# ChuWeiEr/GravInv3DHMC

Measured on AMD Instinct MI355X. Metric: HMC leapfrog steps/sec + G·ρ achieved HBM GB/s at 1/2/4/8 GPUs, higher is better.
Workload: dtype f64

## Files before the change

gravinv3dhmc_amd/_lib.py:

```python
import ctypes as C
import os

import numpy as np

_HERE = os.path.dirname(os.path.abspath(__file__))
LIB_PATH = os.environ.get("GRAVHMC_LIB") or os.path.join(_HERE, "libgravhmc.so")

GH_OK, GH_ERR_ARG, GH_ERR_HIP, GH_ERR_NOMEM, GH_ERR_OVERFLOW, GH_ERR_UNSUPPORTED, GH_ERR_COMM = \
    0, -1, -2, -3, -4, -5, -6
CELL_PRISM, CELL_TESSEROID, CELL_PRISM_TF, CELL_PRISM_COMP, CELL_TESSEROID_COMP, CELL_PRISM_JOINT = 0, 1, 2, 3, 4, 5
CELL_PRISM_MULTI = 6
CELL_PRISM_MVI = 7
CELL_PRISM_MVI_DATA = 8
CELL_TESS_MVI_DATA = 9
CELL_TESSEROID_MULTI = 10
BCOMP_TF, BCOMP_BX, BCOMP_BY, BCOMP_BZ = range(4)
BCOMPONENTS = {"tf": BCOMP_TF, "bx": BCOMP_BX, "by": BCOMP_BY, "bz": BCOMP_BZ}
BCOMP_MAX = 4
MULTI_MAX = 11
COMP_POTENTIAL, COMP_GEOID, COMP_GX, COMP_GY, COMP_GZ, COMP_GXX, COMP_GXY, COMP_GXZ, COMP_GYY, COMP_GYZ, COMP_GZZ = \
    range(11)
COMPONENTS = {"potential": COMP_POTENTIAL, "geoid": COMP_GEOID, "gx": COMP_GX, "gy": COMP_GY, "gz": COMP_GZ,
              "gxx": COMP_GXX, "gxy": COMP_GXY, "gxz": COMP_GXZ, "gyy": COMP_GYY, "gyz": COMP_GYZ, "gzz": COMP_GZZ}
REG_KINDS = {"Damping": 0, "Smoothness": 1, "MS": 2, "TV": 3}
# ... 111 lines not shown
    "gh_shard_init_callback": (C.c_int, [_ctx, C.c_void_p, C.c_void_p, C.c_int, C.c_int, _i64, _i64]),
    "gh_shard_init_rows": (C.c_int, [_ctx, C.c_void_p, C.c_int, C.c_int, _i64, _i64]),
    "gh_shard_init_rows_callback": (C.c_int, [_ctx, C.c_void_p, C.c_void_p, C.c_int, C.c_int, _i64, _i64]),
    "gh_shard_allreduce": (C.c_int, [_ctx, _dp, _i64]),
    "gh_rng_create": (C.c_int, [C.POINTER(C.c_void_p), C.c_uint32]),
    "gh_rng_destroy": (None, [C.c_void_p]),
    "gh_rng_set_threads": (C.c_int, [C.c_void_p, C.c_int]),
    "gh_host_cores": (C.c_int, []),
    "gh_rng_set_state": (C.c_int, [C.c_void_p, C.POINTER(C.c_uint32), C.c_int, C.c_int, C.c_double]),
    "gh_rng_get_state": (C.c_int, [C.c_void_p, C.POINTER(C.c_uint32), C.POINTER(C.c_int), C.POINTER(C.c_int),
                                   C.POINTER(C.c_double)]),
    "gh_rng_draw_trajectories": (C.c_int, [C.c_void_p, C.c_int, C.c_int, C.c_int, _i64, C.c_double,
                                           C.POINTER(C.c_int), _dp, _dp]),
    "gh_format_row_fixed8": (C.c_int64, [_dp, _i64, C.c_char_p, _i64]),
    "gh_measure_stream_read": (C.c_int, [_ctx, C.c_int, C.c_int, C.POINTER(C.c_double)]),
    "gh_profile_enable": (C.c_int, [_ctx, C.c_int]),
    "gh_fold_info": (C.c_int, [_ctx, C.POINTER(C.c_int), C.POINTER(C.c_int), C.POINTER(_i64), C.POINTER(C.c_double),
                               C.POINTER(C.c_double)]),
    "gh_fold_detect": (C.c_int, [_i64, _dp, _dp, _dp, _i64, _dp, C.POINTER(C.c_int), C.POINTER(C.c_int)]),
    "gh_fold_pair_info": (C.c_int, [_ctx, C.POINTER(C.c_int), C.POINTER(C.c_int), C.POINTER(_i64), C.POINTER(_i64),
                                    C.POINTER(_i64)]),
    "gh_fold_detect_pair": (C.c_int, [_i64, _dp, _dp, _dp, _i64, _dp, C.POINTER(C.c_int), C.POINTER(C.c_int),
                                      C.POINTER(C.c_int), C.POINTER(_i64), C.POINTER(C.c_int)]),
    "gh_profile_read": (C.c_int, [_ctx, C.POINTER(C.c_double), C.POINTER(_i64),
                                  C.POINTER(_i64)]),
    "gh_set_translation_invariant": (C.c_int, [_ctx, C.c_int]),
    "gh_translation_invariant_info": (C.c_int, [_ctx] + [C.POINTER(C.c_int)] * 6 + [C.POINTER(_i64), C.POINTER(C.c_double),
                                                                                   C.POINTER(C.c_double)]),
    "gh_translation_invariant_table": (C.c_int, [_ctx, _dp]),
    "gh_lattice_detect": (C.c_int, [_i64, _dp, _dp, _dp, _i64, _dp] + [C.POINTER(C.c_int)] * 5),
}

ALLREDUCE_FN = C.CFUNCTYPE(C.c_int, C.c_void_p, _dp, _i64)

_LIB = None


class GravHmcError(RuntimeError):
    pass


def load():
    global _LIB
    if _LIB is None:
        if not os.path.exists(LIB_PATH):
            raise GravHmcError(
# ... 41 lines not shown
```

gravinv3dhmc_amd/csrc/fold.hip.h:

```cpp
#pragma once

namespace ghk {

struct FoldArgs {
    const double *S;
    const int *obs_img;
    const int *cell_orbit;
    int nF, ldF;
    int64_t n_orb;
    int64_t orb_per_team;
    int n_pp;
    int64_t N;
};

typedef const d2 __attribute__((address_space(1))) *gconst_d2ptr;

__global__ void __launch_bounds__(256) fold_build_kernel(const double *G, int64_t ld, FoldArgs f, double *S,
                                                         unsigned long long *dev_bits)
{
    __shared__ double red[2][4];
    const int64_t o = blockIdx.x;
    const int n = 4 * f.ldF;
    int co[4];
#pragma unroll
// ... 266 lines not shown
            const int e = k * TT + tid;
            const double p2 = __shfl_xor(acc[k][1].x, 1, WAVE), p3 = __shfl_xor(acc[k][1].y, 1, WAVE);
            const double tA = acc[k][0].x + p2, tB = acc[k][0].y + p3;
            const int i = e >> 1;
            if (e < n2 && i < f.nF) {
                const int m2 = 2 * (tid & 1);
                out[f.obs_img[4 * i + m2]] = tA;
                out[f.obs_img[4 * i + m2 + 1]] = tB;
                ds += tA;
                ds += tB;
            }
        }
        for (int64_t e = f.N + tid; e < a.ld; e += TT) out[e] = 0.0;
        if (a.dsum) {
            const double t = block_allreduce_sum(ds, scratch, NW);
            if (tid == 0) a.dsum[blockIdx.x] = t;
        }
    }
}


struct FoldPairArgs {
    const int *wtab;
    const int *obs_img_tau;
    int64_t n_work, work_per_team;
};
constexpr int FOLD_PAIR_W = 16;
constexpr int FOLD_PSLOT = 64;

__global__ void __launch_bounds__(256) fold_pair_mean_kernel(FoldArgs f, const int *row_tau, const int *orb_tau, double *S,
                                                             unsigned long long *dev_bits)
{
    __shared__ double red[2][4];
    const int64_t o = blockIdx.x;
    const int ot = orb_tau[o];
    const int64_t o2 = ot >> 2;
    const int co = ot & 3;
    const int n = 4 * f.nF;
    const int64_t ldb = 4 * (int64_t)f.ldF;
    double dev = 0.0, amax = 0.0;
    if (o <= o2) {
        for (int e = threadIdx.x; e < n; e += blockDim.x) {
            const int k = e & 3, rt = row_tau[e >> 2];
            const int ks = ((k & 1) << 1) | (k >> 1);
            const int e2 = (rt & ~3) | (ks ^ co ^ (rt & 3));
            if (o < o2 || e < e2) {
                const double u = S[o * ldb + e], v = S[o2 * ldb + e2];
                const double m = (u + v) * 0.5;
                S[o * ldb + e] = m;
                S[o2 * ldb + e2] = m;
                dev = fmax(dev, fabs(u - m));
// ... 17 lines not shown
    if (threadIdx.x == 0) {
        for (int w = 1; w < (int)(blockDim.x >> 6); ++w) {
            dev = fmax(dev, red[0][w]);
            amax = fmax(amax, red[1][w]);
        }
        const double rel = amax > 0.0 ? dev / amax : 0.0;
        atomicMax(dev_bits, (unsigned long long)__double_as_longlong(rel));
    }
}

template <int ROWS>
struct FoldPairCol {
    d2 v[ROWS][2];
    int j;
    int jn, on;
    bool live;
    double cv;
};

template <int ROWS>
__global__ void __launch_bounds__(512) fold_pair_sweep_kernel(SweepArgs a, FoldArgs f, FoldPairArgs p)
{
    constexpr int TT = 512, NW = 8;
    extern __shared__ __attribute__((aligned(16))) double smem[];
    double *rF = smem;
    double *rT = smem + 4 * f.nF;
    double *scratch = smem + 8 * f.nF;

    const int tid = threadIdx.x;
    const int lane = tid & 63;
    const int wave = tid >> 6;
    const int mode = a.mode;

    if (mode & SW_ADJ) {
        for (int e = tid; e < 4 * f.nF; e += TT) {
            rF[e] = a.r[f.obs_img[e]];
            rT[e] = a.r[p.obs_img_tau[e]];
        }
    }
    __syncthreads();

    const int64_t wb = (int64_t)blockIdx.x * p.work_per_team;
    int64_t wend = wb + p.work_per_team;
    if (wend > p.n_work) wend = p.n_work;
    const int cnt = wb < wend ? (int)(wend - wb) : 0;

    d2 acc[ROWS][2], accT[ROWS][2];
#pragma unroll
    for (int k = 0; k < ROWS; ++k) acc[k][0] = acc[k][1] = accT[k][0] = accT[k][1] = d2{0.0, 0.0};
    double pp = 0.0;

    const int row_last = (ROWS - 1) * TT + tid;
    const bool last_in = row_last < f.nF;
    unsigned voff = (unsigned)tid * 32u;
    unsigned coff_last = (unsigned)(row_last < f.ldF ? row_last : f.ldF - 1) * 32u;
    const int lrow_last = last_in ? row_last : f.nF - 1;

    const int hl = (lane >> 3) & 3, ql = lane & 7, sl = lane >> 5;
    const double *in_base = ql == FOLD_IN_P      ? a.p_in
                            : ql == FOLD_IN_GREG ? a.greg
                            : ql == FOLD_IN_HI   ? a.high
                            : ql == FOLD_IN_LO   ? a.low
                            : ql == FOLD_IN_PN   ? a.pn_in
                            : (ql == FOLD_IN_GACC && (mode & SW_GACC)) ? a.g_out
                                                                       : a.x_in;
    const int lastc = cnt - 1;
    auto item = [&](int i) -> int64_t { return wb + (i < lastc ? i : lastc); };
    auto load_col = [&](FoldPairCol<ROWS> &c, int64_t w_after) {
        const int jn = p.wtab[FOLD_PAIR_W * w_after + (lane >> 3)];
        const int on = p.wtab[FOLD_PAIR_W * w_after + 8];
        const int64_t o = __builtin_amdgcn_readfirstlane(c.on);
        const unsigned long long col = (unsigned long long)(f.S + o * (int64_t)(4 * f.ldF));
#pragma unroll
        for (int k = 0; k < ROWS - 1; ++k) {
            unsigned long long colk = col + (unsigned long long)k * TT * 32u;
            asm volatile("" : "+s"(colk));
            asm volatile("" : "+v"(voff));
            c.v[k][0] = __builtin_nontemporal_load(reinterpret_cast<gconst_d2ptr>(colk + voff));
            c.v[k][1] = __builtin_nontemporal_load(reinterpret_cast<gconst_d2ptr>(colk + voff) + 1);
        }
        asm volatile("" : "+v"(coff_last));
        c.v[ROWS - 1][0] = __builtin_nontemporal_load(reinterpret_cast<gconst_d2ptr>(col + coff_last));
        c.v[ROWS - 1][1] = __builtin_nontemporal_load(reinterpret_cast<gconst_d2ptr>(col + coff_last) + 1);
        asm volatile("" : "+v"(c.jn)::"memory");
        c.live = c.jn >= 0;
        c.j = c.live ? c.jn : ~c.jn;
        c.cv = in_base[c.j];
        c.jn = jn;
        c.on = on;
    };

    auto row_fma = [](const d2 v0, const d2 v1, const d2 wa, const d2 wb2, d2 &t01, d2 &t23) {
        t01.x += v0.x * wa.x;
        t01.x += v0.y * wa.y;
        t01.x += v1.x * wb2.x;
        t01.x += v1.y * wb2.y;
        t01.y += v0.x * wa.y;
        t01.y += v0.y * wa.x;
        t01.y += v1.x * wb2.y;
        t01.y += v1.y * wb2.x;
        t23.x += v0.x * wb2.x;
        t23.x += v0.y * wb2.y;
        t23.x += v1.x * wa.x;
        t23.x += v1.y * wa.y;
        t23.y += v0.x * wb2.y;
        t23.y += v0.y * wb2.x;
        t23.y += v1.x * wa.y;
        t23.y += v1.y * wa.x;
    };

    auto process = [&](const FoldPairCol<ROWS> &cur, int it) {
        double xl = cur.cv;
        const double pl = dpp_from_up<FOLD_IN_P>(cur.cv);
        if (mode & SW_ADJ) {
            const d2 *r2 = reinterpret_cast<const d2 *>(rF), *t2 = reinterpret_cast<const d2 *>(rT);
            d2 ua = d2{0.0, 0.0}, ub = ua, uta = ua, utb = ua;
#pragma unroll
            for (int k = 0; k < ROWS; ++k) {
                if (k < ROWS - 1 || last_in) {
                    const int row = k < ROWS - 1 ? k * TT + tid : lrow_last;
                    row_fma(cur.v[k][0], cur.v[k][1], r2[2 * row], r2[2 * row + 1], ua, ub);
                    row_fma(cur.v[k][0], cur.v[k][1], t2[2 * row], t2[2 * row + 1], uta, utb);
                }
            }
            const bool odd = (lane & 1) != 0, hi2 = (lane & 2) != 0;
            const double u[4] = {ua.x, ua.y, ub.x, ub.y}, ut[4] = {uta.x, uta.y, utb.x, utb.y};
            double b[4];
#pragma unroll
            for (int q = 0; q < 4; ++q) b[q] = (odd ? ut[q] : u[q]) + dpp_mov<0xb1>(odd ? u[q] : ut[q]);
            double s0 = (hi2 ? b[2] : b[0]) + dpp_mov<0x4e>(hi2 ? b[0] : b[2]);
            double s1 = (hi2 ? b[3] : b[1]) + dpp_mov<0x4e>(hi2 ? b[1] : b[3]);
            s0 = dpp_add<0x114, 0xf>(s0);
            s0 = dpp_add<0x118, 0xf>(s0);
            s1 = dpp_add<0x114, 0xf>(s1);
            s1 = dpp_add<0x118, 0xf>(s1);
            s0 += __shfl_xor(s0, 16, WAVE);
            s1 += __shfl_xor(s1, 16, WAVE);
            s0 += __shfl_xor(s0, 32, WAVE);
            s1 += __shfl_xor(s1, 32, WAVE);
            double *slot = scratch + (it & 1) * FOLD_PSLOT;
            if (lane >= 12 && lane < 16) {
                const int c = lane - 12;
                *reinterpret_cast<d2 *>(slot + wave * 8 + 4 * (c & 1) + 2 * (c >> 1)) = d2{s0, s1};
            }
            __syncthreads();
            double sv = slot[lane];
            sv = dpp_add<0x118, 0xf>(sv);
            sv += __shfl_xor(sv, 16, WAVE);
            sv += __shfl_xor(sv, 32, WAVE);
// ... 22 lines not shown
            if (mode & SW_PFIN) {
                const double pz = cur.live ? pf : 0.0;
#pragma unroll
                for (int h = 0; h < 8; ++h) {
                    const double q = readlane_d(pz, 8 * h);
                    pp += q * q;
                }
            }
            if (tid < 64 && ql == 0 && cur.live) {
                const int j = cur.j;
                if (mode & SW_GOUT) a.g_out[j] = (mode & SW_GACC) ? dpp_from_up<FOLD_IN_GACC>(cur.cv) + g : g;
                if (mode & SW_UPD) {
                    a.p_out[j] = pv;
                    a.x_out[j] = xl;
                } else if ((mode & SW_PFIN) && !(mode & SW_SPEC)) {
                    a.p_out[j] = pv;
                }
            }
        }
        if (mode & SW_FWD) {
            const double xz = cur.live ? xl : 0.0;
            const d2 xa = d2{readlane_d(xz, 0), readlane_d(xz, 8)}, xb = d2{readlane_d(xz, 16), readlane_d(xz, 24)};
            const d2 ya = d2{readlane_d(xz, 32), readlane_d(xz, 40)}, yb = d2{readlane_d(xz, 48), readlane_d(xz, 56)};
#pragma unroll
            for (int k = 0; k < ROWS; ++k) {
                row_fma(cur.v[k][0], cur.v[k][1], xa, xb, acc[k][0], acc[k][1]);
                row_fma(cur.v[k][0], cur.v[k][1], ya, yb, accT[k][0], accT[k][1]);
            }
        }
#pragma unroll
        for (int k = 0; k < ROWS; ++k) {
            asm volatile("" ::"v"(cur.v[k][0]));
            asm volatile("" ::"v"(cur.v[k][1]));
        }
    };

    if (cnt > 0) {
        FoldPairCol<ROWS> b0, b1;
        b0.jn = p.wtab[FOLD_PAIR_W * item(0) + (lane >> 3)];
        b0.on = p.wtab[FOLD_PAIR_W * item(0) + 8];
        b1.jn = p.wtab[FOLD_PAIR_W * item(1) + (lane >> 3)];
        b1.on = p.wtab[FOLD_PAIR_W * item(1) + 8];
        load_col(b0, item(2));
        int i = 0;
        for (;;) {
            load_col(b1, item(i + 3));
            process(b0, i);
            if (++i >= cnt) break;
            load_col(b0, item(i + 3));
            process(b1, i);
            if (++i >= cnt) break;
        }
    }

    if ((mode & SW_PFIN) && tid == 0) {
        a.pp_part[blockIdx.x] = pp;
        for (int t = (int)(blockIdx.x + gridDim.x); t < f.n_pp; t += (int)gridDim.x) a.pp_part[t] = 0.0;
    }

    if (mode & SW_FWD) {
        double *out = a.slab + (int64_t)blockIdx.x * a.ld;
        double ds = 0.0;
#pragma unroll
        for (int k = 0; k < ROWS; ++k) {
            const int i = k * TT + tid;
            if (i < f.nF) {
                const int4 oi = reinterpret_cast<const int4 *>(f.obs_img)[i];
                out[oi.x] = acc[k][0].x;
                out[oi.y] = acc[k][0].y;
                out[oi.z] = acc[k][1].x;
                out[oi.w] = acc[k][1].y;
                ds += acc[k][0].x;
                ds += acc[k][0].y;
                ds += acc[k][1].x;
                ds += acc[k][1].y;
            }
        }
        for (int64_t e = f.N + tid; e < a.ld; e += TT) out[e] = 0.0;
        __syncthreads();
#pragma unroll
        for (int k = 0; k < ROWS; ++k) {
            const int i = k * TT + tid;
            if (i < f.nF) {
                const int4 oi = reinterpret_cast<const int4 *>(p.obs_img_tau)[i];
                out[oi.x] += accT[k][0].x;
                out[oi.y] += accT[k][0].y;
                out[oi.z] += accT[k][1].x;
                out[oi.w] += accT[k][1].y;
                ds += accT[k][0].x;
                ds += accT[k][0].y;
                ds += accT[k][1].x;
                ds += accT[k][1].y;
            }
        }
        if (a.dsum) {
            const double t = block_allreduce_sum(ds, scratch, NW);
            if (tid == 0) a.dsum[blockIdx.x] = t;
        }
    }
}

}
```

gravinv3dhmc_amd/csrc/gravhmc.hip:

```cpp
#include "../../include/gravhmc.h"
#include "kernels.hip.h"
#include "batch.hip.h"
#include "bscg.hip.h"
#include "exchange.hip.h"
#include "resident.hip.h"
#include "resbatch.hip.h"
#include "teamsweep.hip.h"
#include "mfbatch.hip.h"
#include "batchteam.hip.h"
#include "lonsym.hip.h"
#include "lonsymh.hip.h"
#include "lonres.hip.h"
#include "lonsymw.hip.h"
#include "fold.hip.h"
#include "lattice.hip.h"
#include "poststream.hip.h"
#include "tessmag.hip.h"

#include <dlfcn.h>
#include <rccl/rccl.h>

#include <algorithm>
#include <array>
#include <atomic>
// ... 2407 lines not shown
    return GH_OK;
}

int gh_fold_detect_pair(int64_t N, const double *x, const double *y, const double *z, int64_t M, const double *bounds6,
                        int *obs_tau, int *cell_tau, int *work, int64_t *n_work, int *pair_reason)
{
    if (N < 0 || M < 0 || !x || !y || !z || !bounds6 || !obs_tau || !cell_tau || !work || !n_work || !pair_reason)
        return GH_ERR_ARG;
    std::vector<int> oi, co, ot, ct, rt, qt, wk;
    *n_work = 0;
    *pair_reason = GH_FOLD_PAIR_NO_FOLD;
    const int rc = fold_detect_host(N, x, y, z, M, bounds6, oi, co);
    if (rc != GH_FOLD_ON) return rc;
    *pair_reason = fold_pair_detect_host(N, x, y, z, M, bounds6, oi, co, ot, ct, rt, qt, wk);
    if (*pair_reason == GH_FOLD_PAIR_ON) {
        std::copy(ot.begin(), ot.end(), obs_tau);
        std::copy(ct.begin(), ct.end(), cell_tau);
        std::copy(wk.begin(), wk.end(), work);
        *n_work = (int64_t)(wk.size() / 2);
    }
    return rc;
}

int gh_fold_detect(int64_t N, const double *x, const double *y, const double *z, int64_t M, const double *bounds6,
                   int *obs_img, int *cell_orbit)
{
    if (N < 0 || M < 0 || !x || !y || !z || !bounds6 || !obs_img || !cell_orbit) return GH_ERR_ARG;
    std::vector<int> oi, co;
    const int rc = fold_detect_host(N, x, y, z, M, bounds6, oi, co);
    if (rc == GH_FOLD_ON) {
        std::copy(oi.begin(), oi.end(), obs_img);
        std::copy(co.begin(), co.end(), cell_orbit);
    }
    return rc;
}

int gh_profile_read(gh_ctx *c, double *sweep_ms, int64_t *sweep_launches, int64_t *bytes_per_sweep)
{
    if (!c) return GH_ERR_ARG;
    HIPCHK(c, hipSetDevice(c->device));
    HIPCHK(c, hipStreamSynchronize(c->stream));
    const int64_t full = c->N * c->M * (int64_t)sizeof(double);
    int64_t maxb = c->prof_res_evals > 0 ? full : 0;
    for (size_t i = 0; i < c->ev_used / 2; ++i) maxb = std::max(maxb, c->ev_bytes[i]);
    double ms = (c->prof_res_evals > 0 && maxb == full) ? c->prof_ms_acc : 0.0;
    int64_t timed = (c->prof_res_evals > 0 && maxb == full) ? c->prof_res_evals : 0;
// ... 23 lines not shown
```

gravinv3dhmc_amd/csrc/host_ctx.h:

```cpp
#pragma once

static thread_local std::string g_create_error;

struct LonSymHost;
struct LatticeHost;

struct DevBuf {
    void *p = nullptr;
    size_t bytes = 0;
};

struct ExchangeGuard {
    unsigned *abort_w = nullptr;
    unsigned seen[4] = {0, 0, 0, 0};
    unsigned tag = 0, tagE = 0, ltag = 0;
    std::vector<DevBuf> grans;
    bool dirty = false;
    bool inflight = false;
    int aborts = 0;
};

struct BatchSet { double *X, *GREG, *D, *Rt; };

struct gh_ctx {
// ... 291 lines not shown
    uint64_t G_gen = 0;
    struct Fold {
        int detected = 0;
        int reason = GH_FOLD_UNDECIDED;
        uint64_t gen = ~0ull;
        bool valid = false;
        int nF = 0, ldF = 0;
        int64_t n_orb = 0;
        std::vector<int> obs_img, cell_orbit;
        int *obs_img_d = nullptr, *cell_orbit_d = nullptr;
        double *S = nullptr;
        double *zeros = nullptr;
        unsigned long long *dev_bits = nullptr;
        int ept2 = 0, grid = 0;
        int64_t orb_per_team = 0;
        size_t lds = 0;
        double max_dev = 0.0, build_ms = 0.0;
        int64_t launches = 0;
        bool exact = false;
        bool pair_detected = false, pair_on = false;
        int pair_reason = GH_FOLD_PAIR_UNDECIDED;
        int64_t n_work = 0, n_pairs = 0, work_per_team = 0;
        int pair_rows = 0;
        int *wtab_d = nullptr, *obs_img_tau_d = nullptr, *row_tau_d = nullptr, *orb_tau_d = nullptr;
    } fd;

    struct Pinned {
        char *base;
        size_t bytes;
    };
    std::vector<Pinned> pinned;

    double *ring = nullptr, *ring_mean = nullptr, *ring_sd = nullptr;
    int ring_K = 0, ring_next = 0;
    int64_t ring_count = 0;

    struct PostStream {
        bool on = false;
        int slot = 0;
        int64_t from = 0, count = 0;
        ghk::PostState d = {};
        double *lo = nullptr, *hi = nullptr, *iw = nullptr;
        double *row = nullptr;
        double *out = nullptr;
        double *qout = nullptr;
        size_t qout_n = 0;
        int64_t n[16] = {}, K[16] = {};
// ... 114 lines not shown
```

gravinv3dhmc_amd/csrc/host_fold.h:

```cpp
#pragma once


namespace fold_detail {

struct Axis {
    std::vector<double> lo, hi;
    double tol = 0.0;
    void build(std::vector<double> v, double t)
    {
        tol = t;
        std::sort(v.begin(), v.end());
        for (double x : v) {
            if (lo.empty() || x - hi.back() > tol) {
                lo.push_back(x);
                hi.push_back(x);
            } else {
                hi.back() = x;
            }
        }
    }
    int find(double x) const
    {
        const size_t k = (size_t)(std::upper_bound(lo.begin(), lo.end(), x + tol) - lo.begin());
        if (k == 0) return -1;
// ... 230 lines not shown
            if (tau[(size_t)tau[(size_t)i]] != i) return false;
            const int at = pos[(size_t)tau[(size_t)i]] ^ (((g & 1) << 1) | (g >> 1));
            if (g == 0) rt[e >> 2] = at;
            if (rt[e >> 2] != at) return false;
        }
        return true;
    };
    if (!rows(obs_img, obs_tau, row_tau)) return GH_FOLD_PAIR_OBS;
    if (!rows(cell_orbit, cell_tau, orb_tau)) return GH_FOLD_PAIR_CELLS;
    work.clear();
    for (size_t o = 0; o < orb_tau.size(); ++o) {
        const int o2 = orb_tau[o] >> 2;
        if (o2 == (int)o) {
            work.push_back((int)o);
            work.push_back(-1);
        } else if ((int)o < o2) {
            work.push_back((int)o);
            work.push_back(o2);
        }
    }
    return GH_FOLD_PAIR_ON;
}

static int fold_pair_tables(gh_ctx *c, const double *ox, const double *oy, const double *oz, const double *b6)
{
    gh_ctx::Fold &f = c->fd;
    std::vector<int> obs_tau, cell_tau, row_tau, orb_tau, work;
    f.pair_on = false;
    f.n_work = f.n_pairs = 0;
    f.pair_reason = fold_pair_detect_host(c->N, ox, oy, oz, c->M, b6, f.obs_img, f.cell_orbit, obs_tau, cell_tau, row_tau,
                                          orb_tau, work);
    f.pair_detected = f.pair_reason == GH_FOLD_PAIR_ON;
    if (!f.pair_detected) return GH_OK;
    f.pair_reason = GH_FOLD_PAIR_UNDECIDED;
    f.n_work = (int64_t)(work.size() / 2);
    std::vector<int> wtab((size_t)f.n_work * ghk::FOLD_PAIR_W, 0), oit((size_t)c->N);
    for (int64_t w = 0; w < f.n_work; ++w) {
        const int o = work[2 * (size_t)w], o2 = work[2 * (size_t)w + 1];
        int *t = wtab.data() + w * ghk::FOLD_PAIR_W;
        for (int h = 0; h < 4; ++h) {
            t[h] = f.cell_orbit[4 * (size_t)o + h];
            t[4 + h] = o2 >= 0 ? cell_tau[(size_t)t[h]] : ~t[h];
        }
        t[8] = o;
        f.n_pairs += o2 >= 0;
    }
    for (size_t e = 0; e < oit.size(); ++e) oit[e] = obs_tau[(size_t)f.obs_img[e]];
    auto up = [&](int **d, const std::vector<int> &h, size_t cap) -> int {
        TRY(dalloc(c, d, cap, false));
        HIPCHK(c, hipMemcpyAsync(*d, h.data(), sizeof(int) * h.size(), hipMemcpyHostToDevice, c->stream));
        return GH_OK;
    };
    TRY(up(&f.wtab_d, wtab, (size_t)f.n_orb * ghk::FOLD_PAIR_W));
    TRY(up(&f.obs_img_tau_d, oit, (size_t)c->N));
    TRY(up(&f.row_tau_d, row_tau, (size_t)f.nF));
    TRY(up(&f.orb_tau_d, orb_tau, (size_t)f.n_orb));
    HIPCHK(c, hipStreamSynchronize(c->stream));
    return GH_OK;
}

static int fold_detect(gh_ctx *c)
{
    gh_ctx::Fold &f = c->fd;
    f.detected = -1;
    f.valid = false;
    f.gen = ~0ull;
    f.reason = GH_FOLD_NOT_GZ;
    f.pair_detected = f.pair_on = false;
    f.pair_reason = GH_FOLD_PAIR_NO_FOLD;
    if (c->cell_kind != GH_CELL_PRISM || c->joint || c->mf || !c->G) return GH_OK;
    std::vector<double> ox((size_t)c->N), oy((size_t)c->N), oz((size_t)c->N), b6((size_t)c->M * 6);
    TRY(d2h(c, ox.data(), c->obs[0], ox.size()));
    TRY(d2h(c, oy.data(), c->obs[1], oy.size()));
    TRY(d2h(c, oz.data(), c->obs[2], oz.size()));
    TRY(d2h(c, b6.data(), c->bounds, b6.size()));
    f.reason = fold_detect_host(c->N, ox.data(), oy.data(), oz.data(), c->M, b6.data(), f.obs_img, f.cell_orbit);
    if (f.reason != GH_FOLD_ON) return GH_OK;
// ... 26 lines not shown
    case 3: return fold_sweep_kernel<3>;
    case 4: return fold_sweep_kernel<4>;
    case 5: return fold_sweep_kernel<5>;
    }
    return nullptr;
}

typedef void (*fold_pair_fn)(SweepArgs, FoldArgs, FoldPairArgs);

static fold_pair_fn fold_pair_kernel_for(int rows)
{
    switch (rows) {
    case 1: return fold_pair_sweep_kernel<1>;
    case 2: return fold_pair_sweep_kernel<2>;
    case 3: return fold_pair_sweep_kernel<3>;
    case 4: return fold_pair_sweep_kernel<4>;
    case 5: return fold_pair_sweep_kernel<5>;
    }
    return nullptr;
}

constexpr size_t FOLD_PAIR_MAX_LDS = 160u << 10;

static size_t fold_pair_lds(const gh_ctx *c)
{
    return ((size_t)8 * c->fd.nF + 2 * FOLD_PSLOT) * sizeof(double);
}

static int64_t fold_store_bytes(const gh_ctx *c)
{
    return c->fd.n_orb * 4 * (int64_t)c->fd.ldF * (int64_t)sizeof(double);
}

static FoldArgs fold_args(const gh_ctx *c)
{
    const gh_ctx::Fold &f = c->fd;
    FoldArgs a{};
    a.S = f.S;
    a.obs_img = f.obs_img_d;
    a.cell_orbit = f.cell_orbit_d;
    a.nF = f.nF;
    a.ldF = f.ldF;
    a.n_orb = f.n_orb;
    a.orb_per_team = f.orb_per_team;
    a.n_pp = c->n_teams;
    a.N = c->N;
    return a;
}

static FoldPairArgs fold_pair_args(const gh_ctx *c)
{
    const gh_ctx::Fold &f = c->fd;
    FoldPairArgs p{};
    p.wtab = f.wtab_d;
    p.obs_img_tau = f.obs_img_tau_d;
    p.n_work = f.n_work;
    p.work_per_team = f.work_per_team;
    return p;
}

static int64_t fold_sweep_bytes(const gh_ctx *c)
{
    const gh_ctx::Fold &f = c->fd;
    return (f.pair_on ? f.n_work : f.n_orb) * 4 * (int64_t)f.ldF * (int64_t)sizeof(double);
}

static int fold_build(gh_ctx *c)
{
    gh_ctx::Fold &f = c->fd;
    const auto t0 = std::chrono::steady_clock::now();
    TRY(dalloc(c, &f.S, (size_t)(fold_store_bytes(c) / (int64_t)sizeof(double)), false));
    TRY(dalloc(c, &f.dev_bits, 1, false));
    TRY(dalloc(c, &f.zeros, (size_t)c->M));
    HIPCHK(c, hipMemsetAsync(f.dev_bits, 0, sizeof(unsigned long long), c->stream));
    fold_build_kernel<<<dim3((unsigned)f.n_orb), dim3(256), 0, c->stream>>>(c->G, c->ld, fold_args(c), f.S, f.dev_bits);
    HIPCHK(c, hipGetLastError());
    unsigned long long bits = 0;
    HIPCHK(c, hipMemcpyAsync(&bits, f.dev_bits, sizeof bits, hipMemcpyDeviceToHost, c->stream));
    HIPCHK(c, hipStreamSynchronize(c->stream));
    memcpy(&f.max_dev, &bits, sizeof bits);
    if (f.pair_on) {
        HIPCHK(c, hipMemsetAsync(f.dev_bits, 0, sizeof(unsigned long long), c->stream));
        fold_pair_mean_kernel<<<dim3((unsigned)f.n_orb), dim3(256), 0, c->stream>>>(fold_args(c), f.row_tau_d, f.orb_tau_d, f.S,
                                                                                   f.dev_bits);
        HIPCHK(c, hipGetLastError());
        HIPCHK(c, hipMemcpyAsync(&bits, f.dev_bits, sizeof bits, hipMemcpyDeviceToHost, c->stream));
        HIPCHK(c, hipStreamSynchronize(c->stream));
        double d8 = 0.0;
        memcpy(&d8, &bits, sizeof bits);
        f.max_dev += d8;
    }
    f.build_ms = std::chrono::duration<double, std::milli>(std::chrono::steady_clock::now() - t0).count();
    return GH_OK;
}

static int fold_use(gh_ctx *c, bool *use)
{
    gh_ctx::Fold &f = c->fd;
    *use = false;
    if (f.detected != 1 || f.exact) return GH_OK;
    if (c->sh.kind != 0 || c->wv.on || c->joint || c->mf || c->n_panels != 1) {
        f.reason = GH_FOLD_PATH;
        return GH_OK;
    }
    if (f.gen == c->G_gen) {
        *use = f.valid;
        return GH_OK;
    }
    f.gen = c->G_gen;
    f.valid = false;
    f.pair_on = false;
    if (env_int("GRAVHMC_FOLD", 1) == 0) {
        f.reason = GH_FOLD_SWITCHED_OFF;
// ... 2 lines not shown
    const int64_t min_mb = env_int("GRAVHMC_FOLD_MIN_MB", 512);
    if (c->ld * c->M * (int64_t)sizeof(double) <= (min_mb << 20)) {
        f.reason = GH_FOLD_SMALL;
        return GH_OK;
    }
    f.ept2 = (2 * f.ldF + 1023) / 1024;
    if (f.ept2 > FOLD_MAX_EPT2 || (c->ld <= 1024 && env_int("GRAVHMC_RESIDENT", 1) != 0)) {
        f.reason = GH_FOLD_PATH;
        return GH_OK;
    }
    {
        size_t free_b = 0, total_b = 0;
        (void)hipMemGetInfo(&free_b, &total_b);
        if (!f.S && (int64_t)free_b < fold_store_bytes(c) + ((int64_t)256 << 20)) {
            f.reason = GH_FOLD_NOMEM;
            return GH_OK;
        }
    }
    f.pair_on = false;
    f.pair_rows = (f.ldF + 511) / 512;
    if (!f.pair_detected) {
    } else if (env_int("GRAVHMC_FOLD_PAIR", 1) == 0) {
        f.pair_reason = GH_FOLD_PAIR_SWITCHED_OFF;
    } else if (fold_pair_lds(c) > FOLD_PAIR_MAX_LDS || f.pair_rows > FOLD_MAX_EPT2) {
        f.pair_reason = GH_FOLD_PAIR_ROWS;
    } else if (allow_dynamic_lds(reinterpret_cast<const void *>(fold_pair_kernel_for(f.pair_rows)), fold_pair_lds(c)) !=
               hipSuccess) {
        (void)hipGetLastError();
        f.pair_reason = GH_FOLD_PAIR_ROWS;
    } else {
        f.pair_on = true;
        f.pair_reason = GH_FOLD_PAIR_ON;
    }
    const void *fn = f.pair_on ? reinterpret_cast<const void *>(fold_pair_kernel_for(f.pair_rows))
                               : reinterpret_cast<const void *>(fold_kernel_for(f.ept2));
    const int threads = f.pair_on ? 512 : 1024;
    f.lds = f.pair_on ? fold_pair_lds(c) : ((size_t)4 * f.ldF + 2 * FOLD_SLOT) * sizeof(double);
    HIPCHK(c, allow_dynamic_lds(fn, f.lds));
    int occ = 0;
    if (hipOccupancyMaxActiveBlocksPerMultiprocessor(&occ, fn, threads, f.lds) != hipSuccess || occ < 1) {
        (void)hipGetLastError();
        occ = 1;
    }
    const int64_t items = f.pair_on ? f.n_work : f.n_orb;
    int grid = (int)std::min<int64_t>(std::min<int64_t>((int64_t)c->cus * occ, c->grid), items);
    const int64_t per_team = (items + grid - 1) / grid;
    f.orb_per_team = f.work_per_team = per_team;
// ... 46 lines not shown
```

include/gravhmc.h:

```cpp
#ifndef GRAVHMC_H
#define GRAVHMC_H

#include <stdint.h>

#ifdef __cplusplus
extern "C" {
#endif

typedef struct gh_ctx gh_ctx;

typedef enum {
    GH_OK = 0,
    GH_ERR_ARG = -1,
    GH_ERR_HIP = -2,
    GH_ERR_NOMEM = -3,
    GH_ERR_OVERFLOW = -4,
    GH_ERR_UNSUPPORTED = -5,
    GH_ERR_COMM = -6
} gh_status;

enum { GH_CELL_PRISM = 0, GH_CELL_TESSEROID = 1, GH_CELL_PRISM_TF = 2, GH_CELL_PRISM_COMP = 3, GH_CELL_TESSEROID_COMP = 4,
       GH_CELL_PRISM_JOINT = 5, GH_CELL_PRISM_MULTI = 6, GH_CELL_PRISM_MVI = 7, GH_CELL_PRISM_MVI_DATA = 8 };
enum { GH_CELL_TESS_MVI_DATA = 9, GH_CELL_TESSEROID_MULTI = 10 };
enum { GH_BCOMP_TF = 0, GH_BCOMP_BX = 1, GH_BCOMP_BY = 2, GH_BCOMP_BZ = 3 };
// ... 177 lines not shown
    GH_FOLD_FIXED = 6,
    GH_FOLD_SMALL = 7,
    GH_FOLD_PATH = 8,
    GH_FOLD_NOMEM = 9,
    GH_FOLD_DEVIATION = 10
};
int gh_fold_info(const gh_ctx *ctx, int *on, int *reason, int64_t *store_bytes, double *max_dev, double *build_ms);
int gh_fold_detect(int64_t N, const double *x, const double *y, const double *z, int64_t M, const double *bounds6,
                   int *obs_img, int *cell_orbit);

enum {
    GH_FOLD_PAIR_ON = 0,
    GH_FOLD_PAIR_UNDECIDED = 1,
    GH_FOLD_PAIR_SWITCHED_OFF = 2,
    GH_FOLD_PAIR_NO_FOLD = 3,
    GH_FOLD_PAIR_OBS = 4,
    GH_FOLD_PAIR_CELLS = 5,
    GH_FOLD_PAIR_ROWS = 6
};
int gh_fold_pair_info(const gh_ctx *ctx, int *on, int *reason, int64_t *pairs, int64_t *single_orbits,
                      int64_t *bytes_per_sweep);
int gh_fold_detect_pair(int64_t N, const double *x, const double *y, const double *z, int64_t M, const double *bounds6,
                        int *obs_tau, int *cell_tau, int *work, int64_t *n_work, int *pair_reason);


int gh_set_translation_invariant(gh_ctx *ctx, int enable);
int gh_translation_invariant_info(const gh_ctx *ctx, int *on, int *nx, int *ny, int *nz, int *px, int *qy,
                                  int64_t *table_bytes, double *max_dev, double *build_ms);
int gh_translation_invariant_table(gh_ctx *ctx, double *out);
enum {
    GH_LATTICE_ON = 0,
    GH_LATTICE_CELLS = 1,
    GH_LATTICE_HEIGHTS = 2,
    GH_LATTICE_SPACING = 3,
    GH_LATTICE_RECT = 4,
    GH_LATTICE_DUPLICATE = 5,
    GH_LATTICE_DEVIATION = 6,
    GH_LATTICE_LDS = 7
};
int gh_lattice_detect(int64_t N, const double *x, const double *y, const double *z, int64_t M, const double *bounds6,
                      int *dims5, int *lat_of_cell, int *cell_of_lat, int *lat_of_obs, int *obs_of_lat);


int gh_profile_enable(gh_ctx *ctx, int enable);
int gh_profile_read(gh_ctx *ctx, double *sweep_ms, int64_t *sweep_launches,
                    int64_t *bytes_per_sweep);
// ... 8 lines not shown
```

Baseline: 831.7.

## Reorder folded-pair sensitivity rows so tau-paired rows share slots in sweep

```diff
diff --git a/gravinv3dhmc_amd/_lib.py b/gravinv3dhmc_amd/_lib.py
--- a/gravinv3dhmc_amd/_lib.py
+++ b/gravinv3dhmc_amd/_lib.py
@@ -157,6 +157,8 @@
                                     C.POINTER(_i64)]),
     "gh_fold_detect_pair": (C.c_int, [_i64, _dp, _dp, _dp, _i64, _dp, C.POINTER(C.c_int), C.POINTER(C.c_int),
                                       C.POINTER(C.c_int), C.POINTER(_i64), C.POINTER(C.c_int)]),
+    "gh_fold_pair_rows": (C.c_int, [_i64, _dp, _dp, _dp, _i64, _dp, C.POINTER(C.c_int), C.POINTER(C.c_int),
+                                    C.POINTER(C.c_int), C.POINTER(C.c_int), C.POINTER(_i64), C.POINTER(C.c_int)]),
     "gh_profile_read": (C.c_int, [_ctx, C.POINTER(C.c_double), C.POINTER(_i64),
                                   C.POINTER(_i64)]),
     "gh_set_translation_invariant": (C.c_int, [_ctx, C.c_int]),
diff --git a/gravinv3dhmc_amd/csrc/fold.hip.h b/gravinv3dhmc_amd/csrc/fold.hip.h
--- a/gravinv3dhmc_amd/csrc/fold.hip.h
+++ b/gravinv3dhmc_amd/csrc/fold.hip.h
@@ -312,11 +312,28 @@
 
 struct FoldPairArgs {
     const int *wtab;
-    const int *obs_img_tau;
+    const int *ptab;
     int64_t n_work, work_per_team;
 };
 constexpr int FOLD_PAIR_W = 16;
 constexpr int FOLD_PSLOT = 64;
+
+constexpr int fold_pair_slots(int rows) { return (rows - 1) / 2; }
+constexpr int fold_pair_cols(int rows) { return 2 * (rows - fold_pair_slots(rows)); }
+
+__global__ void __launch_bounds__(512) fold_pair_rows_kernel(FoldArgs f, const int *code, double *S)
+{
+    extern __shared__ __attribute__((aligned(16))) double smem[];
+    const int n = 4 * f.ldF;
+    double *blk = S + (int64_t)blockIdx.x * n;
+    for (int e = threadIdx.x; e < n; e += blockDim.x) smem[e] = blk[e];
+    __syncthreads();
+    for (int e = threadIdx.x; e < n; e += blockDim.x) {
+        const int cd = code[e >> 2];
+        const int k = e >> 11, t = (e >> 2) & 511, w = min(512, f.ldF - 512 * k);
+        blk[2048 * k + 2 * (((e >> 1) & 1) * w + t) + (e & 1)] = cd >= 0 ? smem[(cd & ~3) | ((e ^ cd) & 3)] : 0.0;
+    }
+}
 
 __global__ void __launch_bounds__(256) fold_pair_mean_kernel(FoldArgs f, const int *row_tau, const int *orb_tau, double *S,
                                                              unsigned long long *dev_bits)
@@ -380,10 +397,10 @@
 __global__ void __launch_bounds__(512) fold_pair_sweep_kernel(SweepArgs a, FoldArgs f, FoldPairArgs p)
 {
     constexpr int TT = 512, NW = 8;
+    constexpr int NP = fold_pair_slots(ROWS), NS = ROWS - NP, NC = fold_pair_cols(ROWS);
     extern __shared__ __attribute__((aligned(16))) double smem[];
-    double *rF = smem;
-    double *rT = smem + 4 * f.nF;
-    double *scratch = smem + 8 * f.nF;
+    double *rL = smem;
+    double *scratch = smem + NC * TT * 4;
 
     const int tid = threadIdx.x;
     const int lane = tid & 63;
@@ -391,9 +408,9 @@
     const int mode = a.mode;
 
     if (mode & SW_ADJ) {
-        for (int e = tid; e < 4 * f.nF; e += TT) {
-            rF[e] = a.r[f.obs_img[e]];
-            rT[e] = a.r[p.obs_img_tau[e]];
+        for (int e = tid; e < NC * TT * 4; e += TT) {
+            const int i = p.ptab[e];
+            rL[e] = i >= 0 ? a.r[i] : 0.0;
         }
     }
     __syncthreads();
@@ -403,16 +420,16 @@
     if (wend > p.n_work) wend = p.n_work;
     const int cnt = wb < wend ? (int)(wend - wb) : 0;
 
-    d2 acc[ROWS][2], accT[ROWS][2];
-#pragma unroll
-    for (int k = 0; k < ROWS; ++k) acc[k][0] = acc[k][1] = accT[k][0] = accT[k][1] = d2{0.0, 0.0};
+    d2 acc[NS][2][2];
+#pragma unroll
+    for (int s = 0; s < NS; ++s) acc[s][0][0] = acc[s][0][1] = acc[s][1][0] = acc[s][1][1] = d2{0.0, 0.0};
     double pp = 0.0;
 
     const int row_last = (ROWS - 1) * TT + tid;
-    const bool last_in = row_last < f.nF;
-    unsigned voff = (unsigned)tid * 32u;
-    unsigned coff_last = (unsigned)(row_last < f.ldF ? row_last : f.ldF - 1) * 32u;
-    const int lrow_last = last_in ? row_last : f.nF - 1;
+    const bool last_in = row_last < f.ldF;
+    const int w_last = f.ldF - (ROWS - 1) * TT;
+    unsigned voff = (unsigned)tid * 16u;
+    unsigned coff_last = (unsigned)(last_in ? tid : w_last - 1) * 16u;
 
     const int hl = (lane >> 3) & 3, ql = lane & 7, sl = lane >> 5;
     const double *in_base = ql == FOLD_IN_P      ? a.p_in
@@ -425,27 +442,30 @@
     const int lastc = cnt - 1;
     auto item = [&](int i) -> int64_t { return wb + (i < lastc ? i : lastc); };
     auto load_col = [&](FoldPairCol<ROWS> &c, int64_t w_after) {
-        const int jn = p.wtab[FOLD_PAIR_W * w_after + (lane >> 3)];
-        const int on = p.wtab[FOLD_PAIR_W * w_after + 8];
+        asm volatile("" : "+v"(c.jn), "+v"(c.on)::"memory");
         const int64_t o = __builtin_amdgcn_readfirstlane(c.on);
+        c.live = c.jn >= 0;
+        c.j = c.live ? c.jn : ~c.jn;
+        asm volatile("" : "+v"(c.j));
+        c.jn = p.wtab[FOLD_PAIR_W * w_after + (lane >> 3)];
+        c.on = p.wtab[FOLD_PAIR_W * w_after + 8];
         const unsigned long long col = (unsigned long long)(f.S + o * (int64_t)(4 * f.ldF));
 #pragma unroll
         for (int k = 0; k < ROWS - 1; ++k) {
-            unsigned long long colk = col + (unsigned long long)k * TT * 32u;
+            unsigned long long colk = col + (unsigned long long)k * TT * 32u, colh = colk + TT * 16u;
             asm volatile("" : "+s"(colk));
+            asm volatile("" : "+s"(colh));
             asm volatile("" : "+v"(voff));
             c.v[k][0] = __builtin_nontemporal_load(reinterpret_cast<gconst_d2ptr>(colk + voff));
-            c.v[k][1] = __builtin_nontemporal_load(reinterpret_cast<gconst_d2ptr>(colk + voff) + 1);
-        }
+            c.v[k][1] = __builtin_nontemporal_load(reinterpret_cast<gconst_d2ptr>(colh + voff));
+        }
+        unsigned long long coll = col + (unsigned long long)(ROWS - 1) * TT * 32u, collh = coll + (unsigned)w_last * 16u;
+        asm volatile("" : "+s"(coll));
+        asm volatile("" : "+s"(collh));
         asm volatile("" : "+v"(coff_last));
-        c.v[ROWS - 1][0] = __builtin_nontemporal_load(reinterpret_cast<gconst_d2ptr>(col + coff_last));
-        c.v[ROWS - 1][1] = __builtin_nontemporal_load(reinterpret_cast<gconst_d2ptr>(col + coff_last) + 1);
-        asm volatile("" : "+v"(c.jn)::"memory");
-        c.live = c.jn >= 0;
-        c.j = c.live ? c.jn : ~c.jn;
+        c.v[ROWS - 1][0] = __builtin_nontemporal_load(reinterpret_cast<gconst_d2ptr>(coll + coff_last));
+        c.v[ROWS - 1][1] = __builtin_nontemporal_load(reinterpret_cast<gconst_d2ptr>(collh + coff_last));
         c.cv = in_base[c.j];
-        c.jn = jn;
-        c.on = on;
     };
 
     auto row_fma = [](const d2 v0, const d2 v1, const d2 wa, const d2 wb2, d2 &t01, d2 &t23) {
@@ -471,18 +491,26 @@
         double xl = cur.cv;
         const double pl = dpp_from_up<FOLD_IN_P>(cur.cv);
         if (mode & SW_ADJ) {
-            const d2 *r2 = reinterpret_cast<const d2 *>(rF), *t2 = reinterpret_cast<const d2 *>(rT);
-            d2 ua = d2{0.0, 0.0}, ub = ua, uta = ua, utb = ua;
-#pragma unroll
-            for (int k = 0; k < ROWS; ++k) {
+            const d2 *r2 = reinterpret_cast<const d2 *>(rL) + 2 * tid;
+            d2 ua = d2{0.0, 0.0}, ub = ua, wa = ua, wb = ua;
+#pragma unroll
+            for (int s = 0; s < NS; ++s) {
+                const int k = s < NP ? 2 * s : NP + s;
                 if (k < ROWS - 1 || last_in) {
-                    const int row = k < ROWS - 1 ? k * TT + tid : lrow_last;
-                    row_fma(cur.v[k][0], cur.v[k][1], r2[2 * row], r2[2 * row + 1], ua, ub);
-                    row_fma(cur.v[k][0], cur.v[k][1], t2[2 * row], t2[2 * row + 1], uta, utb);
+                    const d2 ra0 = r2[4 * s * TT], ra1 = r2[4 * s * TT + 1];
+                    const d2 rb0 = r2[(4 * s + 2) * TT], rb1 = r2[(4 * s + 2) * TT + 1];
+                    const d2 a0 = cur.v[k][0], a1 = cur.v[k][1];
+                    row_fma(a0, a1, ra0, ra1, ua, ub);
+                    row_fma(d2{a0.x, a1.x}, d2{a0.y, a1.y}, rb0, rb1, wa, wb);
+                    if (s < NP) {
+                        const d2 b0 = cur.v[k + 1][0], b1 = cur.v[k + 1][1];
+                        row_fma(b0, b1, rb0, rb1, ua, ub);
+                        row_fma(d2{b0.x, b1.x}, d2{b0.y, b1.y}, ra0, ra1, wa, wb);
+                    }
                 }
             }
             const bool odd = (lane & 1) != 0, hi2 = (lane & 2) != 0;
-            const double u[4] = {ua.x, ua.y, ub.x, ub.y}, ut[4] = {uta.x, uta.y, utb.x, utb.y};
+            const double u[4] = {ua.x, ua.y, ub.x, ub.y}, ut[4] = {wa.x, wb.x, wa.y, wb.y};
             double b[4];
 #pragma unroll
             for (int q = 0; q < 4; ++q) b[q] = (odd ? ut[q] : u[q]) + dpp_mov<0xb1>(odd ? u[q] : ut[q]);
@@ -551,10 +579,18 @@
             const double xz = cur.live ? xl : 0.0;
             const d2 xa = d2{readlane_d(xz, 0), readlane_d(xz, 8)}, xb = d2{readlane_d(xz, 16), readlane_d(xz, 24)};
             const d2 ya = d2{readlane_d(xz, 32), readlane_d(xz, 40)}, yb = d2{readlane_d(xz, 48), readlane_d(xz, 56)};
-#pragma unroll
-            for (int k = 0; k < ROWS; ++k) {
-                row_fma(cur.v[k][0], cur.v[k][1], xa, xb, acc[k][0], acc[k][1]);
-                row_fma(cur.v[k][0], cur.v[k][1], ya, yb, accT[k][0], accT[k][1]);
+            const d2 ysa = d2{ya.x, yb.x}, ysb = d2{ya.y, yb.y};
+#pragma unroll
+            for (int s = 0; s < NS; ++s) {
+                const int k = s < NP ? 2 * s : NP + s;
+                const d2 a0 = cur.v[k][0], a1 = cur.v[k][1];
+                row_fma(a0, a1, xa, xb, acc[s][0][0], acc[s][0][1]);
+                row_fma(d2{a0.x, a1.x}, d2{a0.y, a1.y}, ysa, ysb, acc[s][1][0], acc[s][1][1]);
+                if (s < NP) {
+                    const d2 b0 = cur.v[k + 1][0], b1 = cur.v[k + 1][1];
+                    row_fma(b0, b1, xa, xb, acc[s][1][0], acc[s][1][1]);
+                    row_fma(d2{b0.x, b1.x}, d2{b0.y, b1.y}, ysa, ysb, acc[s][0][0], acc[s][0][1]);
+                }
             }
         }
 #pragma unroll
@@ -565,21 +601,26 @@
     };
 
     if (cnt > 0) {
-        FoldPairCol<ROWS> b0, b1;
+        FoldPairCol<ROWS> b0, b1, b2;
         b0.jn = p.wtab[FOLD_PAIR_W * item(0) + (lane >> 3)];
         b0.on = p.wtab[FOLD_PAIR_W * item(0) + 8];
         b1.jn = p.wtab[FOLD_PAIR_W * item(1) + (lane >> 3)];
         b1.on = p.wtab[FOLD_PAIR_W * item(1) + 8];
-        load_col(b0, item(2));
+        b2.jn = p.wtab[FOLD_PAIR_W * item(2) + (lane >> 3)];
+        b2.on = p.wtab[FOLD_PAIR_W * item(2) + 8];
+        load_col(b0, item(3));
+        load_col(b1, item(4));
         int i = 0;
-        for (;;) {
-            load_col(b1, item(i + 3));
+        for (; i + 2 < cnt; i += 3) {
+            load_col(b2, item(i + 5));
             process(b0, i);
-            if (++i >= cnt) break;
-            load_col(b0, item(i + 3));
-            process(b1, i);
-            if (++i >= cnt) break;
-        }
+            load_col(b0, item(i + 6));
+            process(b1, i + 1);
+            load_col(b1, item(i + 7));
+            process(b2, i + 2);
+        }
+        if (i < cnt) process(b0, i);
+        if (i + 1 < cnt) process(b1, i + 1);
     }
 
     if ((mode & SW_PFIN) && tid == 0) {
@@ -589,37 +630,39 @@
 
     if (mode & SW_FWD) {
         double *out = a.slab + (int64_t)blockIdx.x * a.ld;
+        const int4 *pt = reinterpret_cast<const int4 *>(p.ptab) + tid;
         double ds = 0.0;
 #pragma unroll
-        for (int k = 0; k < ROWS; ++k) {
-            const int i = k * TT + tid;
-            if (i < f.nF) {
-                const int4 oi = reinterpret_cast<const int4 *>(f.obs_img)[i];
-                out[oi.x] = acc[k][0].x;
-                out[oi.y] = acc[k][0].y;
-                out[oi.z] = acc[k][1].x;
-                out[oi.w] = acc[k][1].y;
-                ds += acc[k][0].x;
-                ds += acc[k][0].y;
-                ds += acc[k][1].x;
-                ds += acc[k][1].y;
+        for (int c = 0; c < NC; ++c) {
+            if ((c & 1) && (c >> 1) >= NP) continue;
+            const int4 oi = pt[c * TT];
+            if (oi.x >= 0) {
+                const d2 s01 = acc[c >> 1][c & 1][0], s23 = acc[c >> 1][c & 1][1];
+                out[oi.x] = s01.x;
+                out[oi.y] = s01.y;
+                out[oi.z] = s23.x;
+                out[oi.w] = s23.y;
+                ds += s01.x;
+                ds += s01.y;
+                ds += s23.x;
+                ds += s23.y;
             }
         }
         for (int64_t e = f.N + tid; e < a.ld; e += TT) out[e] = 0.0;
         __syncthreads();
 #pragma unroll
-        for (int k = 0; k < ROWS; ++k) {
-            const int i = k * TT + tid;
-            if (i < f.nF) {
-                const int4 oi = reinterpret_cast<const int4 *>(p.obs_img_tau)[i];
-                out[oi.x] += accT[k][0].x;
-                out[oi.y] += accT[k][0].y;
-                out[oi.z] += accT[k][1].x;
-                out[oi.w] += accT[k][1].y;
-                ds += accT[k][0].x;
-                ds += accT[k][0].y;
-                ds += accT[k][1].x;
-                ds += accT[k][1].y;
+        for (int s = NP; s < NS; ++s) {
+            const int4 oi = pt[(2 * s + 1) * TT];
+            if (oi.x >= 0) {
+                const d2 s01 = acc[s][1][0], s23 = acc[s][1][1];
+                out[oi.x] += s01.x;
+                out[oi.y] += s01.y;
+                out[oi.z] += s23.x;
+                out[oi.w] += s23.y;
+                ds += s01.x;
+                ds += s01.y;
+                ds += s23.x;
+                ds += s23.y;
             }
         }
         if (a.dsum) {
diff --git a/gravinv3dhmc_amd/csrc/gravhmc.hip b/gravinv3dhmc_amd/csrc/gravhmc.hip
--- a/gravinv3dhmc_amd/csrc/gravhmc.hip
+++ b/gravinv3dhmc_amd/csrc/gravhmc.hip
@@ -2453,6 +2453,34 @@
     return rc;
 }
 
+int gh_fold_pair_rows(int64_t N, const double *x, const double *y, const double *z, int64_t M, const double *bounds6,
+                      int *rows, int *pair_slots, int *code, int *ptab, int64_t *counts, int *pair_reason)
+{
+    if (N < 0 || M < 0 || !x || !y || !z || !bounds6 || !rows || !pair_slots || !code || !ptab || !counts || !pair_reason)
+        return GH_ERR_ARG;
+    std::vector<int> oi, co, ot, ct, rt, qt, wk;
+    *rows = *pair_slots = 0;
+    *pair_reason = GH_FOLD_PAIR_NO_FOLD;
+    const int rc = fold_detect_host(N, x, y, z, M, bounds6, oi, co);
+    if (rc != GH_FOLD_ON) return rc;
+    *pair_reason = fold_pair_detect_host(N, x, y, z, M, bounds6, oi, co, ot, ct, rt, qt, wk);
+    if (*pair_reason != GH_FOLD_PAIR_ON) return rc;
+    const int nF = (int)(N / 4), ldF = (nF + 15) / 16 * 16;
+    fold_detail::PairRows pr;
+    if (ldF > 512 * FOLD_PAIR_MAX_ROWS || !fold_detail::pair_rows_plan(nF, ldF, oi, rt, pr)) {
+        *pair_reason = GH_FOLD_PAIR_ROWS;
+        return rc;
+    }
+    *rows = pr.rows;
+    *pair_slots = pr.pair_slots;
+    std::copy(pr.code.begin(), pr.code.end(), code);
+    std::copy(pr.ptab.begin(), pr.ptab.end(), ptab);
+    counts[0] = pr.pairs_in_slots;
+    counts[1] = pr.pairs_split;
+    counts[2] = pr.self_rows;
+    return rc;
+}
+
 int gh_fold_detect(int64_t N, const double *x, const double *y, const double *z, int64_t M, const double *bounds6,
                    int *obs_img, int *cell_orbit)
 {
diff --git a/gravinv3dhmc_amd/csrc/host_ctx.h b/gravinv3dhmc_amd/csrc/host_ctx.h
--- a/gravinv3dhmc_amd/csrc/host_ctx.h
+++ b/gravinv3dhmc_amd/csrc/host_ctx.h
@@ -337,7 +337,9 @@
         int pair_reason = GH_FOLD_PAIR_UNDECIDED;
         int64_t n_work = 0, n_pairs = 0, work_per_team = 0;
         int pair_rows = 0;
-        int *wtab_d = nullptr, *obs_img_tau_d = nullptr, *row_tau_d = nullptr, *orb_tau_d = nullptr;
+        bool pair_rows_ok = false;
+        int *wtab_d = nullptr, *row_tau_d = nullptr, *orb_tau_d = nullptr;
+        int *ptab_d = nullptr, *row_code_d = nullptr;
     } fd;
 
     struct Pinned {
diff --git a/gravinv3dhmc_amd/csrc/host_fold.h b/gravinv3dhmc_amd/csrc/host_fold.h
--- a/gravinv3dhmc_amd/csrc/host_fold.h
+++ b/gravinv3dhmc_amd/csrc/host_fold.h
@@ -276,6 +276,68 @@
     return GH_FOLD_PAIR_ON;
 }
 
+namespace fold_detail {
+
+struct PairRows {
+    int rows = 0, pair_slots = 0, cols = 0;
+    int64_t pairs_in_slots = 0, pairs_split = 0, self_rows = 0;
+    std::vector<int> code, ptab;
+};
+
+inline bool pair_rows_plan(int nF, int ldF, const std::vector<int> &obs_img, const std::vector<int> &row_tau, PairRows &pr)
+{
+    constexpr int TT = 512;
+    pr.rows = (ldF + TT - 1) / TT;
+    pr.pair_slots = ghk::fold_pair_slots(pr.rows);
+    pr.cols = ghk::fold_pair_cols(pr.rows);
+    pr.pairs_in_slots = pr.pairs_split = pr.self_rows = 0;
+    pr.code.assign((size_t)ldF, -1);
+    pr.ptab.assign((size_t)pr.cols * TT * 4, -1);
+    auto place = [&](int s, int t, int k, int f, bool both) {
+        const int rt = row_tau[(size_t)f], f2 = rt >> 2, cf = rt & 3;
+        int *pa = pr.ptab.data() + ((size_t)(2 * s) * TT + (size_t)t) * 4, *pb = pa + (size_t)TT * 4;
+        for (int g = 0; g < 4; ++g) {
+            pa[g] = obs_img[4 * (size_t)f + g];
+            pb[g] = obs_img[4 * (size_t)f2 + (g ^ cf)];
+        }
+        pr.code[(size_t)k * TT + t] = 4 * f;
+        if (both) pr.code[(size_t)(k + 1) * TT + t] = 4 * f2 + cf;
+    };
+    const int64_t cap = (int64_t)pr.pair_slots * TT;
+    int64_t lone = 0;
+    auto place_lone = [&](int f) -> bool {
+        const int64_t n = 2 * cap + lone;
+        if (n >= ldF) return false;
+        const int l = (int)(lone / TT), t = (int)(lone % TT);
+        place(pr.pair_slots + l, t, 2 * pr.pair_slots + l, f, false);
+        ++lone;
+        return true;
+    };
+    int64_t np = 0;
+    for (int f = 0; f < nF; ++f) {
+        const int f2 = row_tau[(size_t)f] >> 2;
+        if (f2 <= f) continue;
+        if (np < cap) {
+            place((int)(np / TT), (int)(np % TT), 2 * (int)(np / TT), f, true);
+            ++pr.pairs_in_slots;
+        } else {
+            if (!place_lone(f) || !place_lone(f2)) return false;
+            ++pr.pairs_split;
+        }
+        ++np;
+    }
+    for (int f = 0; f < nF; ++f) {
+        if ((row_tau[(size_t)f] >> 2) != f) continue;
+        if (!place_lone(f)) return false;
+        ++pr.self_rows;
+    }
+    return true;
+}
+
+}
+
+constexpr int FOLD_PAIR_MAX_ROWS = 5;
+
 static int fold_pair_tables(gh_ctx *c, const double *ox, const double *oy, const double *oz, const double *b6)
 {
     gh_ctx::Fold &f = c->fd;
@@ -288,7 +350,7 @@
     if (!f.pair_detected) return GH_OK;
     f.pair_reason = GH_FOLD_PAIR_UNDECIDED;
     f.n_work = (int64_t)(work.size() / 2);
-    std::vector<int> wtab((size_t)f.n_work * ghk::FOLD_PAIR_W, 0), oit((size_t)c->N);
+    std::vector<int> wtab((size_t)f.n_work * ghk::FOLD_PAIR_W, 0);
     for (int64_t w = 0; w < f.n_work; ++w) {
         const int o = work[2 * (size_t)w], o2 = work[2 * (size_t)w + 1];
         int *t = wtab.data() + w * ghk::FOLD_PAIR_W;
@@ -299,14 +361,20 @@
         t[8] = o;
         f.n_pairs += o2 >= 0;
     }
-    for (size_t e = 0; e < oit.size(); ++e) oit[e] = obs_tau[(size_t)f.obs_img[e]];
+    fold_detail::PairRows pr;
+    f.pair_rows_ok = f.ldF <= 512 * FOLD_PAIR_MAX_ROWS && fold_detail::pair_rows_plan(f.nF, f.ldF, f.obs_img, row_tau, pr);
+    if (!f.pair_rows_ok) {
+        pr.code.assign((size_t)f.ldF, -1);
+        pr.ptab.assign(4, -1);
+    }
     auto up = [&](int **d, const std::vector<int> &h, size_t cap) -> int {
         TRY(dalloc(c, d, cap, false));
         HIPCHK(c, hipMemcpyAsync(*d, h.data(), sizeof(int) * h.size(), hipMemcpyHostToDevice, c->stream));
         return GH_OK;
     };
     TRY(up(&f.wtab_d, wtab, (size_t)f.n_orb * ghk::FOLD_PAIR_W));
-    TRY(up(&f.obs_img_tau_d, oit, (size_t)c->N));
+    TRY(up(&f.ptab_d, pr.ptab, (size_t)ghk::fold_pair_cols(FOLD_PAIR_MAX_ROWS) * 512 * 4));
+    TRY(up(&f.row_code_d, pr.code, (size_t)f.ldF));
     TRY(up(&f.row_tau_d, row_tau, (size_t)f.nF));
     TRY(up(&f.orb_tau_d, orb_tau, (size_t)f.n_orb));
     HIPCHK(c, hipStreamSynchronize(c->stream));
@@ -379,9 +447,14 @@
 
 constexpr size_t FOLD_PAIR_MAX_LDS = 160u << 10;
 
+static size_t fold_pair_lds_limit(const gh_ctx *c)
+{
+    return ((size_t)8 * c->fd.nF + 2 * FOLD_PSLOT) * sizeof(double);
+}
+
 static size_t fold_pair_lds(const gh_ctx *c)
 {
-    return ((size_t)8 * c->fd.nF + 2 * FOLD_PSLOT) * sizeof(double);
+    return ((size_t)ghk::fold_pair_cols(c->fd.pair_rows) * 512 * 4 + 2 * FOLD_PSLOT) * sizeof(double);
 }
 
 static int64_t fold_store_bytes(const gh_ctx *c)
@@ -410,7 +483,7 @@
     const gh_ctx::Fold &f = c->fd;
     FoldPairArgs p{};
     p.wtab = f.wtab_d;
-    p.obs_img_tau = f.obs_img_tau_d;
+    p.ptab = f.ptab_d;
     p.n_work = f.n_work;
     p.work_per_team = f.work_per_team;
     return p;
@@ -446,6 +519,11 @@
         double d8 = 0.0;
         memcpy(&d8, &bits, sizeof bits);
         f.max_dev += d8;
+        const size_t blk = (size_t)4 * f.ldF * sizeof(double);
+        HIPCHK(c, allow_dynamic_lds(reinterpret_cast<const void *>(fold_pair_rows_kernel), blk));
+        fold_pair_rows_kernel<<<dim3((unsigned)f.n_orb), dim3(512), blk, c->stream>>>(fold_args(c), f.row_code_d, f.S);
+        HIPCHK(c, hipGetLastError());
+        HIPCHK(c, hipStreamSynchronize(c->stream));
     }
     f.build_ms = std::chrono::duration<double, std::milli>(std::chrono::steady_clock::now() - t0).count();
     return GH_OK;
@@ -494,7 +572,7 @@
     if (!f.pair_detected) {
     } else if (env_int("GRAVHMC_FOLD_PAIR", 1) == 0) {
         f.pair_reason = GH_FOLD_PAIR_SWITCHED_OFF;
-    } else if (fold_pair_lds(c) > FOLD_PAIR_MAX_LDS || f.pair_rows > FOLD_MAX_EPT2) {
+    } else if (fold_pair_lds_limit(c) > FOLD_PAIR_MAX_LDS || f.pair_rows > FOLD_PAIR_MAX_ROWS || !f.pair_rows_ok) {
         f.pair_reason = GH_FOLD_PAIR_ROWS;
     } else if (allow_dynamic_lds(reinterpret_cast<const void *>(fold_pair_kernel_for(f.pair_rows)), fold_pair_lds(c)) !=
                hipSuccess) {
diff --git a/include/gravhmc.h b/include/gravhmc.h
--- a/include/gravhmc.h
+++ b/include/gravhmc.h
@@ -223,6 +223,8 @@
                       int64_t *bytes_per_sweep);
 int gh_fold_detect_pair(int64_t N, const double *x, const double *y, const double *z, int64_t M, const double *bounds6,
                         int *obs_tau, int *cell_tau, int *work, int64_t *n_work, int *pair_reason);
+int gh_fold_pair_rows(int64_t N, const double *x, const double *y, const double *z, int64_t M, const double *bounds6,
+                      int *rows, int *pair_slots, int *code, int *ptab, int64_t *counts, int *pair_reason);
 
 
 int gh_set_translation_invariant(gh_ctx *ctx, int enable);
```

After: 1018 (median of 6 runs). +22.3%, better.
